# dcvan24/pivot-scheduling

Hardware: AMD Instinct MI355X
Metric: task x host placement candidates scored/sec (HBM GB/s % peak) at 1/2/4/8 MI355X (higher is better)
Workload: dtype f64; 1 GPU; synthetic 1000000 hosts x 10000 ready tasks per round, 20 zones, cost_aware best-fit, one independent scenario per GPU; scenarios_per_gpu=1, tasks_per_round=10000, zones=20, policy=ca_bf, parallelism=scenario-sharded x1 (no data-path collective)

## Files before the change

pivot-scheduling_amd/csrc/pvt_zwalk.hip:

```cpp
#include <hip/hip_runtime.h>
#include <stdint.h>

#include "pivot_place.h"
#include "pvt_device.h"
#include "pvt_kernels.h"
#include "pvt_zwin_dev.h"

namespace pvt {

constexpr int ZW_THREADS = 256;
constexpr int ZW_WAVES = ZW_THREADS / 64;
constexpr int ZW_SCAN = 8;
constexpr int ZW_MINB = ZW_MIN_PARTS;
constexpr int ZW_PR = 8;
constexpr double ZW_BIG = 0x1p500;

#ifndef PVT_ZW_UNROLL
#define PVT_ZW_UNROLL 8
#endif
#ifndef PVT_ZW_CF
#define PVT_ZW_CF 0
#endif
constexpr int ZW_UNROLL = PVT_ZW_UNROLL;
constexpr int ZW_SB = 64;
constexpr int32_t ZW_SAME = -1;
template <int WM>
struct ZwalkLDS {
  double wa[4][WM];
  int32_t wid[WM];
  int32_t wz[WM];
  uint64_t zm[WM / 64];
  double csum[ZMAX * ZMAX], bsum[ZMAX * ZMAX];
  int32_t cnt[ZW_SCAN][ZW_WAVES];
  double red[ZW_WAVES][12];
  double smin[ZW_SB][4];
  double lg[128][4];
  int32_t lgid[128];
  int32_t rwho[64], rstart[64];
  uint64_t sbits[CHAIN_MAX / 64];
  uint32_t amask[ZMAX];
  uint32_t umask;
  int32_t nwin, bail;
  int32_t touch[WM / 64];
};

__device__ __forceinline__ double nan_max(double a, double b) {
  return (a != a || b <= a) ? a : b;
}
__device__ __forceinline__ double wave_nmax_d(double v) {
  return wave_reduce_d(v, [](double a, double b) { return nan_max(a, b); });
}

__global__ __launch_bounds__(256) void host_min_kernel(const double* avail, int H, int lo, int hi,
                                                       double* part) {
  __shared__ double red[4][4];
  const int tid = threadIdx.x, lane = tid & 63, wave = tid >> 6;
  double m[4] = {DINF, DINF, DINF, DINF};
  for (int h = lo + blockIdx.x * 256 + tid; h < hi; h += gridDim.x * 256)
#pragma unroll
    for (int r = 0; r < 4; r++) m[r] = fmin(m[r], avail[(size_t)r * H + h]);
#pragma unroll
  for (int r = 0; r < 4; r++) {
    m[r] = wave_min_d(m[r]);
    if (lane == 0) red[wave][r] = m[r];
  }
  __syncthreads();
  if (tid < 4) {
    double v = red[0][tid];
    for (int w = 1; w < 4; w++) v = fmin(v, red[w][tid]);
    part[blockIdx.x * 4 + tid] = v;
  }
}

template <int N> struct IntC { static constexpr int value = N; };

constexpr int ZW_CAP = 128;
__device__ __forceinline__ int lowbit_exp(double v) {
  const uint64_t b = (uint64_t)__double_as_longlong(v);
  const uint64_t m = b & ((1ull << 52) - 1);
  const int e = (int)((b >> 52) & 0x7ff);
  if (e == 0) return m ? -1074 + __builtin_ctzll(m) : 4096;
  return (e - 1075) + __builtin_ctzll(m | (1ull << 52));
}
__device__ __forceinline__ int high_exp(double v) {
  return (int)(((uint64_t)__double_as_longlong(v) >> 52) & 0x7ff) - 1023;
}
template <bool STRICT>
__device__ __forceinline__ int copies_cf(double x, double d, bool& sure) {
  if (__double_as_longlong(d) == 0) return ZW_CAP;
  const double q = x * __builtin_amdgcn_rcp(d);
  double kf = STRICT ? __builtin_ceil(q) - 1.0 : __builtin_floor(q);
  kf = __builtin_fmin(kf, (double)ZW_CAP);
  const double e0 = __builtin_fma(-kf, d, x), e1 = __builtin_fma(-(kf + 1.0), d, x);
  const double big = __builtin_fabs(x) + (kf + 1.0) * d;
  const bool nice = high_exp(big) + 2 <= min(lowbit_exp(x), lowbit_exp(d)) + 53;
  const double err = nice ? 0.0 : (kf + 2.0) * 0x1p-52 * (big + d);
  const bool fit0 = STRICT ? (e0 > err) : (e0 >= err && (nice || e0 > err));
  const bool out1 = kf >= (double)ZW_CAP || (STRICT ? (e1 <= -err && (nice || e1 < -err)) : (e1 < -err));
  sure = sure && kf >= 1.0 && fit0 && out1 && (q == q);
  return (int)kf;
}

#define UNI(c) (__builtin_amdgcn_readfirstlane((int)(c)) != 0)

template <bool STRICT>
__device__ __forceinline__ bool fit_res(double m) { return STRICT ? (m > 0.0) : (m >= 0.0); }

__device__ __forceinline__ void wave_lds_sync() {
  __atomic_signal_fence(__ATOMIC_SEQ_CST);
  __builtin_amdgcn_s_waitcnt(0xc07f);
  __atomic_signal_fence(__ATOMIC_SEQ_CST);
}

template <int WM = ZW_M>
__device__ __forceinline__ void compact_zone_window(const int32_t* zone, int Z, uint32_t U,
                                                    int h_lo, int h_hi, int32_t* wid, int32_t* wz,
                                                    int32_t (*cnt)[ZW_WAVES], int32_t* nwin) {
  compact_zone_window_t<WM, ZW_THREADS, ZW_SCAN>(zone, Z, U, h_lo, h_hi, wid, wz, cnt, nwin);
}

#ifdef PVT_STAMPS
__device__ __forceinline__ uint64_t zstamp() {
  uint64_t t;
  __builtin_amdgcn_sched_barrier(0);
  asm volatile("s_memtime %0\n\ts_waitcnt lgkmcnt(0)" : "=s"(t)::"memory");
  __builtin_amdgcn_sched_barrier(0);
  return t;
}
#endif

template <bool KEYED, bool STRICT, bool FF = false, int WM = ZW_M, bool FAST = false>
__global__ __launch_bounds__(ZW_THREADS) void zwalk_kernel(ZwalkArgs A) {
  static_assert(!FF || (!KEYED && STRICT), "FF: chain mode, strict fit");
  static_assert(WM == ZW_M || !KEYED, "keyed / ordered / sharded windows: ZW_M hosts");
  __shared__ ZwalkLDS<WM> S;
#ifdef PVT_STAMPS
  const uint64_t t_start = zstamp();
  uint64_t n_chunks = 0, n_switch = 0, n_bulk = 0, n_runs = 0;
  uint64_t st_search = 0, st_p1 = 0, st_p2 = 0, n_probe = 0, n_iter = 0, st_batch = 0, n_single = 0;
  uint64_t st_setup = 0, st_loop = 0, st_who = 0, st_rep = 0;
  uint64_t n_cf = 0;
#endif
  const int b = blockIdx.x, tid = threadIdx.x, lane = tid & 63, wave = tid >> 6;
  const bool tabm = !KEYED && A.tab.nch > 0;
  const int base = KEYED ? 0 : tabm ? A.tab.coff[b] : A.coff[b];
  const int nt = KEYED ? A.knt : tabm ? A.tab.coff[b + 1] - A.tab.coff[b] : A.coff[b + 1] - base;
  const int32_t* gcmap = KEYED ? nullptr : A.cmap + base;
  auto cmap_at = [&](int i) -> int { return gcmap[i]; };
  const bool segm = !KEYED && (tabm || A.cseg);
  int32_t* status = A.status + 2 * b;
  const int Z = A.Z, H = A.H;
  auto report = [&](int s0, int s1) {
    status[0] = s0; status[1] = s1;
    if (!KEYED && A.hstat) { A.hstat[2 * b] = s0; A.hstat[2 * b + 1] = s1; }
  };

  auto publish_map = [&]() {
    if (tabm) {
      int32_t* wmap = const_cast<int32_t*>(A.cmap) + base;
      for (int k = A.tab.csoff[b]; k < A.tab.csoff[b + 1]; k++) {
        const int sg = A.tab.csegid[k], c0 = A.tab.seg_cstart[sg], o0 = A.tab.seg_off[sg];
        const int len = A.tab.seg_off[sg + 1] - o0;
        for (int i = tid; i < len; i += ZW_THREADS) wmap[c0 + i] = o0 + i;
      }
      if (b == 0) {
        const int ns = A.tab.nseg, nc = A.tab.nch;
        for (int i = tid; i <= ns; i += ZW_THREADS) {
          A.tab.o_seg_off[i] = A.tab.seg_off[i];
          if (i < ns) { A.tab.o_seg_chain[i] = A.tab.seg_chain[i]; A.tab.o_seg_cstart[i] = A.tab.seg_cstart[i]; }
        }
        for (int i = tid; i <= nc; i += ZW_THREADS) A.tab.o_coff[i] = A.tab.coff[i];
      }
    }
  };
  double mn[4];
  uint32_t U;
  int nwin;
#ifdef PVT_STAMPS
  uint64_t t_load, t_cert, t_win, t_cap;
#endif
  if constexpr (FAST) {
    static_assert(!KEYED && !FF && WM == ZW_M && ZW_M == 4 * ZW_THREADS, "fast prologue: best-fit chains");
    static_assert(ZW_ENT <= 64 && ZW_ENT <= ZW_SB, "entries: a lane each, in rwho / rstart / lg");
    const int j = min((int)A.cert.cwin[b], ZMAX - 1);
    const ZoneWindow* const zw = &A.zpre->w[j];
    const int ZZ = Z * Z;
    double cs[4], bs[4], ha[4];
#pragma unroll
    for (int u = 0; u < 4; u++) {
      const int i = tid + u * ZW_THREADS;
      cs[u] = i < ZZ ? A.csum[i] : 0.0;
      bs[u] = i < ZZ ? A.bsum[i] : 0.0;
    }
#pragma unroll
    for (int r = 0; r < 4; r++) ha[r] = A.hmin[tid * 4 + r];
    const uint32_t zu = A.zpre->U[j];
    const int zn = zw->n, zbad = zw->bad;
    int32_t wi[4], wzv[4];
    double wv[4][4];
#pragma unroll
    for (int u = 0; u < 4; u++) {
      const int p = tid + u * ZW_THREADS;
      wi[u] = zw->id[p];
      wzv[u] = zw->z[p];
#pragma unroll
      for (int r = 0; r < 4; r++) wv[u][r] = zw->a[r][p];
    }
    const int k0 = A.tab.csoff[b], k1 = A.tab.csoff[b + 1];
    double mxv = -DINF;
    bool badv = false;
    for (int k = k0 + wave; k < k1; k += ZW_WAVES) {
      const int sg = A.tab.csegid[k], c0 = A.tab.seg_cstart[sg];
      const int len = A.tab.seg_off[sg + 1] - A.tab.seg_off[sg];
      const GroupCert* const gc = A.cert.rec + min((int)A.cert.seg_grp[sg], GCOMPACT_MAX - 1);
      const int ne = (len + 63) >> 6, e = A.cert.seg_ent[sg] + lane;
      const bool on = lane < ne && lane < GC_SUB && e < ZW_ENT;
      double sm[4];
#pragma unroll
      for (int r = 0; r < 4; r++) sm[r] = on ? gc->smin[lane][r] : DINF;
      const double gm = lane < 4 ? gc->mx[lane] : -DINF;
      badv |= gc->bad != 0 || gc->n != len;
      mxv = fmax(mxv, gm);
      if (on) {
#pragma unroll
        for (int r = 0; r < 4; r++) S.lg[e][r] = sm[r];
        S.rstart[e] = c0 + 64 * lane;
        S.rwho[e] = c0 + min(64 * lane + 64, len);
      }
    }
    publish_map();
#pragma unroll
    for (int u = 0; u < 4; u++) {
      const int i = tid + u * ZW_THREADS;
      if (i < ZZ) { S.csum[i] = cs[u]; S.bsum[i] = bs[u]; }
    }
    if (tid < CHAIN_MAX / 64) S.sbits[tid] = 0;
    if (tid < WM / 64) S.touch[tid] = 0;
    if (tid < ZW_SB) {
#pragma unroll
      for (int r = 0; r < 4; r++) S.smin[tid][r] = -DINF;
    }
    nwin = min(zn, ZW_M);
#pragma unroll
    for (int u = 0; u < 4; u++) {
      const int p = tid + u * ZW_THREADS;
      if (p < nwin) {
        S.wid[p] = wi[u];
        S.wz[p] = wzv[u];
#pragma unroll
        for (int r = 0; r < 4; r++) S.wa[r][p] = wv[u][r];
      }
    }
#pragma unroll
    for (int r = 0; r < 4; r++) ha[r] = wave_min_d(ha[r]);
    const bool wbadv = __ballot(badv) != 0;
    if (lane < 4) S.red[wave][lane] = mxv;
    if (lane == 0) {
#pragma unroll
      for (int r = 0; r < 4; r++) S.red[wave][8 + r] = ha[r];
      S.cnt[0][wave] = wbadv ? 1 : 0;
    }
#ifdef PVT_STAMPS
    t_load = zstamp();
#endif
    __syncthreads();
    if (tid < Z) {
      uint32_t m = 0;
      for (int z = 0; z < Z; z++) m |= (S.csum[tid * Z + z] == 0.0) ? (1u << z) : 0u;
      S.amask[tid] = m;
    }
    for (int k = k0 + tid; k < k1; k += ZW_THREADS) {
      const int p = A.tab.seg_cstart[A.tab.csegid[k]];
      if (p > 0 && p < CHAIN_MAX) atomicOr(&S.sbits[p >> 6], 1ull << (p & 63));
    }
    double mx[4];
    bool bad = false;
#pragma unroll
    for (int w = 0; w < ZW_WAVES; w++) bad |= S.cnt[0][w] != 0;
#pragma unroll
    for (int r = 0; r < 4; r++) {
      mx[r] = fmax(fmax(S.red[0][r], S.red[1][r]), fmax(S.red[2][r], S.red[3][r]));
      ha[r] = fmin(fmin(S.red[0][8 + r], S.red[1][8 + r]), fmin(S.red[2][8 + r], S.red[3][8 + r]));
    }
    const int ne = min((int)A.cert.cent[b], ZW_ENT);
    {
      double v = lane < ne ? S.lg[lane][wave] : DINF;
#pragma unroll
      for (int off = 1; off < 64; off <<= 1) v = fmin(v, __shfl_down(v, off));
      if (lane < ne) {
        const int q = (S.rstart[lane] + 63) >> 6;
        if (q * 64 < S.rwho[lane] && q < ZW_SB) S.smin[q][wave] = v;
      }
      if (lane == 0) S.red[0][4 + wave] = v;
    }
    bool sep = false;
#pragma unroll
    for (int r = 0; r < 4; r++) sep |= (ha[r] - mx[r] >= 0x1p-288);
    U = zu;
    const bool cover = zu != 0 && (A.cert.cu[b] & ~zu) == 0;
    const bool stop = bad || !sep || nt <= 0 || nt > CHAIN_MAX || !cover || zbad != 0 || nwin <= 0;
#ifdef PVT_STAMPS
    t_cert = t_win = t_cap = zstamp();
#endif
    __syncthreads();
    if (tid == 0) {
      int cert = stop ? 0 : ZW_CERT_FAST;
#pragma unroll
      for (int r = 0; r < 4; r++) {
        const double mnr = S.red[0][4 + r];
        cert |= ((mx[r] <= 0.0 && mnr >= 0.0) ? (1 << r) : 0) | ((ha[r] >= 0x1p-287) ? (16 << r) : 0);
      }
      if (A.hcert) A.hcert[b] = cert;
      if (stop) report(0, nt <= 0 ? 0 : 1);
    }
    if (A.cmax && tid < 4) A.cmax[b * 4 + tid] = mx[tid];
    if (stop) return;
  } else {
    static_assert(ZMAX * ZMAX <= 4 * ZW_THREADS && ZW_MINB == ZW_THREADS, "prologue loads");
    const int ZZ = KEYED ? 0 : Z * Z;
    double cs[4], bs[4];
#pragma unroll
    for (int u = 0; u < 4; u++) {
      const int i = tid + u * ZW_THREADS;
      cs[u] = i < ZZ ? A.csum[i] : 0.0;
      bs[u] = i < ZZ ? A.bsum[i] : 0.0;
    }
    double ha[4] = {FF ? -DINF : DINF, FF ? -DINF : DINF, FF ? -DINF : DINF, FF ? -DINF : DINF};
    if (!KEYED) {
#pragma unroll
      for (int r = 0; r < 4; r++) {
        const double x = A.hmin[tid * 4 + r];
        ha[r] = FF ? nan_max(ha[r], x) : fmin(ha[r], x);
      }
    }
    publish_map();
    int wv[ZW_PR];
    if (tabm) {
      const int k0 = A.tab.csoff[b], k1 = A.tab.csoff[b + 1];
#pragma unroll
      for (int u = 0; u < ZW_PR; u++) {
        const int i = u * ZW_THREADS + tid;
        int v = -1;
        for (int k = k0; k < k1; k++) {
          const int sg = A.tab.csegid[k], c0 = A.tab.seg_cstart[sg];
          if (i >= c0) v = A.tab.seg_off[sg] + (i - c0);
        }
        wv[u] = i < nt ? v : -1;
      }
    } else {
#pragma unroll
      for (int u = 0; u < ZW_PR; u++) {
        const int i = u * ZW_THREADS + tid;
        wv[u] = i < nt ? (KEYED ? i : gcmap[i]) : -1;
      }
    }
    const int sg0 = tabm ? A.tab.csoff[b] : (!KEYED && A.cseg) ? A.csoff[b] : 0;
    const int sg1 = tabm ? A.tab.csoff[b + 1] : (!KEYED && A.cseg) ? A.csoff[b + 1] : 0;
    const uint32_t zpu = (!KEYED && WM == ZW_M && A.zpre && lane < Z) ? A.zpre->U[lane] : 0u;

#pragma unroll
    for (int u = 0; u < 4; u++) {
      const int i = tid + u * ZW_THREADS;
      if (i < ZZ) { S.csum[i] = cs[u]; S.bsum[i] = bs[u]; }
    }
    if (tid == 0) { S.umask = 0; S.nwin = 0; S.bail = 0; }
    if (tid < CHAIN_MAX / 64) S.sbits[tid] = 0;
    if (tid < WM / 64) S.touch[tid] = 0;
#ifdef PVT_STAMPS
    t_load = zstamp();
#endif
    __syncthreads();
    if (!KEYED && tid < Z) {
      uint32_t m = 0;
      for (int z = 0; z < Z; z++) m |= (S.csum[tid * Z + z] == 0.0) ? (1u << z) : 0u;
      S.amask[tid] = m;
    }
    if (tabm) {
      for (int k = sg0 + tid; k < sg1; k += ZW_THREADS) {
        const int p = A.tab.seg_cstart[A.tab.csegid[k]];
        if (p > 0 && p < CHAIN_MAX) atomicOr(&S.sbits[p >> 6], 1ull << (p & 63));
      }
    } else {
      for (int k = sg0 + tid; k < sg1; k += ZW_THREADS) {
        const int p = A.cseg[k];
        if (p > 0 && p < CHAIN_MAX) atomicOr(&S.sbits[p >> 6], 1ull << (p & 63));
      }
    }

    uint32_t abits = 0;
    double mx[4] = {-DINF, -DINF, -DINF, -DINF};
    mn[0] = mn[1] = mn[2] = mn[3] = DINF;
    bool bad = false;
    for (int i0 = 0; i0 < nt; i0 += ZW_PR * ZW_THREADS) {
      int av[ZW_PR], wn[ZW_PR];
      double dv[ZW_PR][4];
#pragma unroll
      for (int u = 0; u < ZW_PR; u++) {
        const int w = max(wv[u], 0);
        av[u] = A.anc[w];
#pragma unroll
        for (int r = 0; r < 4; r++) dv[u][r] = A.dem[(size_t)w * 4 + r];
      }
#pragma unroll
      for (int u = 0; u < ZW_PR; u++) {
        const int i = i0 + ZW_PR * ZW_THREADS + u * ZW_THREADS + tid;
        wn[u] = i < nt ? (KEYED ? i : cmap_at(i)) : -1;
      }
#pragma unroll
      for (int u = 0; u < ZW_PR; u++) {
        const bool ok = wv[u] >= 0;
        double bm[4];
#pragma unroll
        for (int r = 0; r < 4; r++) bm[r] = ok ? dv[u][r] : DINF;
        if (ok) {
          const int a = av[u];
          if (a < 0 || a >= Z) {
            bad = true;
          } else {
            abits |= 1u << a;
#pragma unroll
            for (int r = 0; r < 4; r++) {
              bad |= !(__builtin_fabs(dv[u][r]) <= ZW_BIG);
              mx[r] = fmax(mx[r], dv[u][r]);
              mn[r] = fmin(mn[r], dv[u][r]);
            }
          }
        }
        const int blk = (i0 + u * ZW_THREADS) / 64 + wave;
        if (blk < ZW_SB - 1 && blk * 64 < nt) {
#pragma unroll
          for (int r = 0; r < 4; r++) bm[r] = wave_min_d(bm[r]);
          if (lane == 0) {
#pragma unroll
            for (int r = 0; r < 4; r++) S.smin[blk][r] = bm[r];
          }
        }
      }
#pragma unroll
      for (int u = 0; u < ZW_PR; u++) wv[u] = wn[u];
    }
    __syncthreads();
    uint32_t um = 0;
    if (!KEYED)
      for (uint32_t m = abits; m; m &= m - 1) um |= S.amask[__builtin_ctz(m)];
#pragma unroll
    for (int r = 0; r < 4; r++) {
      mx[r] = wave_max_d(mx[r]);
      mn[r] = wave_min_d(mn[r]);
      ha[r] = FF ? wave_nmax_d(ha[r]) : wave_min_d(ha[r]);
    }
    if (lane == 0) {
#pragma unroll
      for (int r = 0; r < 4; r++) { S.red[wave][r] = mx[r]; S.red[wave][4 + r] = mn[r]; S.red[wave][8 + r] = ha[r]; }
    }
    if (bad) S.bail = 1;
    if (um) atomicOr(&S.umask, um);
    __syncthreads();
#ifdef PVT_STAMPS
    t_cert = zstamp();
#endif
#pragma unroll
    for (int r = 0; r < 4; r++) {
      for (int w = 1; w < ZW_WAVES; w++) {
        mx[r] = fmax(mx[r], S.red[w][r]);
        mn[r] = fmin(mn[r], S.red[w][4 + r]);
        ha[r] = FF ? nan_max(ha[r], S.red[w][8 + r]) : fmin(ha[r], S.red[w][8 + r]);
      }
      mx[r] = fmax(mx[r], S.red[0][r]);
      mn[r] = fmin(mn[r], S.red[0][4 + r]);
      ha[r] = FF ? nan_max(ha[r], S.red[0][8 + r]) : fmin(ha[r], S.red[0][8 + r]);
    }
    if (!KEYED && A.cmax && tid < 4) A.cmax[b * 4 + tid] = mx[tid];
    if (!KEYED && A.hcert && tid == 0) {
      int cert = 0;
      if (!FF) {
#pragma unroll
        for (int r = 0; r < 4; r++)
          cert |= ((mx[r] <= 0.0 && mn[r] >= 0.0) ? (1 << r) : 0) | ((ha[r] >= 0x1p-287) ? (16 << r) : 0);
      }
      A.hcert[b] = cert;
    }
    bool sep = KEYED;
    if (FF) {
      sep = true;
#pragma unroll
      for (int r = 0; r < 4; r++) sep &= (ha[r] <= 0x1p298) && (mn[r] >= 0.0);
    } else {
#pragma unroll
      for (int r = 0; r < 4; r++) sep |= (ha[r] - mx[r] >= 0x1p-288);
    }
    U = S.umask;
    if (S.bail || !sep || nt <= 0 || (!KEYED && nt > CHAIN_MAX)) {
      if (tid == 0) report(0, (KEYED || nt <= 0) ? 0 : 1);
      return;
    }
    const FrontierSlot* pw = A.pwin ? A.pwin + (KEYED ? 0 : b) : nullptr;
    const ZoneWindow* zw = nullptr;
    if (!KEYED && WM == ZW_M && !pw && A.zpre && U != 0) {
      const uint64_t cover = __ballot(zpu != 0 && (U & ~zpu) == 0);
      if (cover) {
        const int j = __builtin_ctzll(cover);
        zw = &A.zpre->w[j];
        U = (uint32_t)__builtin_amdgcn_readlane((int)zpu, j);
      }
    }
    if (pw) {
      const int nw = min(pw->n, ZW_M);
      for (int p = tid; p < nw; p += ZW_THREADS) {
        const int32_t h = pw->id[p];
        S.wid[p] = h;
        S.wz[p] = KEYED ? 0 : A.zone[h];
      }
      if (tid == 0) S.nwin = nw;
      __syncthreads();
    } else if (zw) {
      const int nw = min(zw->n, ZW_M);
      for (int p = tid; p < nw; p += ZW_THREADS) { S.wid[p] = zw->id[p]; S.wz[p] = zw->z[p]; }
      if (tid == 0) S.nwin = nw;
      __syncthreads();
    } else if (KEYED) {
      const int nw = min(A.kn_dev ? *A.kn_dev : A.kn, ZW_M);
      for (int p = tid; p < nw; p += ZW_THREADS) { S.wid[p] = A.lo + A.kperm[p]; S.wz[p] = 0; }
      if (tid == 0) S.nwin = nw;
      __syncthreads();
    } else {
      compact_zone_window<WM>(A.zone, Z, U, 0, H, S.wid, S.wz, S.cnt, &S.nwin);
    }
    nwin = S.nwin;
#ifdef PVT_STAMPS
    t_win = zstamp();
#endif
    bool wbad = false;
    ZwUndo* const ud = (!KEYED && A.undo) ? A.undo + b : nullptr;
    if (ud && tid == 0) ud->count = nwin;
    static_assert(WM <= ZW_MBIG, "ZwUndo holds every window");
    static_assert(WM % (4 * ZW_THREADS) == 0, "window capacities: four hosts per thread per pass");
    for (int p0 = 0; p0 < WM && p0 < nwin; p0 += 4 * ZW_THREADS) {
      double v[4][4];
#pragma unroll
      for (int u = 0; u < 4; u++) {
        const int p = p0 + u * ZW_THREADS + tid;
        const int h = p < nwin ? S.wid[p] : 0;
#pragma unroll
        for (int r = 0; r < 4; r++)
          v[u][r] = p >= nwin ? 0.0 : (pw ? pw->a[r][p] : zw ? zw->a[r][p] : A.avail[(size_t)r * H + h]);
      }
#pragma unroll
      for (int u = 0; u < 4; u++) {
        const int p = p0 + u * ZW_THREADS + tid;
        if (p < nwin) {
#pragma unroll
          for (int r = 0; r < 4; r++) {
            wbad |= !(__builtin_fabs(v[u][r]) <= ZW_BIG);
            S.wa[r][p] = v[u][r];
          }
          if (ud) {
            ud->id[p] = S.wid[p];
#pragma unroll
            for (int r = 0; r < 4; r++) ud->a[r][p] = v[u][r];
          }
        }
      }
    }
    if (wbad) S.bail = 1;
    __syncthreads();
#ifdef PVT_STAMPS
    t_cap = zstamp();
#endif
    if (S.bail || nwin == 0) {
      if (tid == 0) report(0, KEYED ? 0 : 1);
      return;
    }
    const int nsb = min((nt + 63) >> 6, ZW_SB);
    for (int blk = ZW_SB - 1 + wave; blk < nsb; blk += ZW_WAVES) {
      const int i1 = blk == ZW_SB - 1 ? nt : min(nt, blk * 64 + 64);
      double bm[4] = {DINF, DINF, DINF, DINF};
      for (int i = blk * 64 + lane; i < i1; i += 64) {
        const int w = KEYED ? i : cmap_at(i);
#pragma unroll
        for (int r = 0; r < 4; r++) bm[r] = fmin(bm[r], A.dem[(size_t)w * 4 + r]);
      }
#pragma unroll
      for (int r = 0; r < 4; r++) bm[r] = wave_min_d(bm[r]);
      if (lane == 0) {
#pragma unroll
        for (int r = 0; r < 4; r++) S.smin[blk][r] = bm[r];
      }
    }
    __syncthreads();
    static_assert(ZW_SB == 64 && ZW_WAVES == 4, "suffix minima: one wave per dimension, a lane per batch");
    {
      double v = lane < nsb ? S.smin[lane][wave] : DINF;
#pragma unroll
      for (int off = 1; off < 64; off <<= 1) v = fmin(v, __shfl_down(v, off));
      if (lane < nsb) S.smin[lane][wave] = v;
    }
    __syncthreads();
  }
  if (wave != 0) return;
#ifdef PVT_STAMPS
  const uint64_t t_walk = zstamp();
#endif

  const int nch = (nwin + 63) >> 6;
  int p0 = 0;
  int cur = -1;
  int done = 0;
  bool failed = false, exhausted = false;
  double ra0, ra1, ra2, ra3;
  int32_t rid;
  uint64_t rzm = 0, rvalid = 0;
  bool dirty = false;
  auto load_chunk = [&](int c) {
    const int p = c * 64 + lane;
    const int q = min(p, nwin - 1);
    ra0 = S.wa[0][q]; ra1 = S.wa[1][q]; ra2 = S.wa[2][q]; ra3 = S.wa[3][q];
    rid = S.wid[q];
    rvalid = __ballot(p < nwin);
    dirty = false;
    __builtin_amdgcn_s_waitcnt(0xc07f);
  };
  auto store_chunk = [&](int c) {
    const int p = c * 64 + lane;
    if (dirty && p < nwin) { S.wa[0][p] = ra0; S.wa[1][p] = ra1; S.wa[2][p] = ra2; S.wa[3][p] = ra3; }
    dirty = false;
  };
  double rb0 = 0.0, rb1 = 0.0, rb2 = 0.0, rb3 = 0.0;
  int32_t bid = 0;
  uint64_t bzm = 0, bvalid = 0;
  bool bdirty = false;
  int pb = -1;
  auto load_b = [&](int c) {
    bdirty = false;
    if (c >= nch) { pb = -1; bvalid = 0; bzm = 0; return; }
    pb = c;
    const int p = c * 64 + lane;
    const int q = min(p, nwin - 1);
    rb0 = S.wa[0][q]; rb1 = S.wa[1][q]; rb2 = S.wa[2][q]; rb3 = S.wa[3][q];
    bid = S.wid[q];
    bvalid = __ballot(p < nwin);
    bzm = cur >= 0 ? rfl_u64(S.zm[c]) : 0;
    __builtin_amdgcn_s_waitcnt(0xc07f);
  };
  auto store_b = [&]() {
    const int p = pb * 64 + lane;
    if (bdirty && pb >= 0 && p < nwin) { S.wa[0][p] = rb0; S.wa[1][p] = rb1; S.wa[2][p] = rb2; S.wa[3][p] = rb3; }
    bdirty = false;
  };
  auto run_bulk = [&](auto cft, double& c0, double& c1, double& c2, double& c3, int32_t cid, double d0,
                      double d1, double d2, double d3, uint64_t m0, int R, int k) -> int {
#ifdef PVT_STAMPS
    const uint64_t tA = zstamp();
#endif
    if (!(d0 >= 0.0 && d1 >= 0.0 && d2 >= 0.0 && d3 >= 0.0)) R = 1;
    const bool on1 = __builtin_amdgcn_inverse_ballot_w64(m0);
    const bool two = __double_as_longlong(d2) == 0 && __double_as_longlong(d3) == 0;
    R = __builtin_amdgcn_readfirstlane(R);
    int cnt = 0;
#ifdef PVT_STAMPS
    const uint64_t tA1 = zstamp();
    st_setup += tA1 - tA;
#endif
    bool cf = false;
#if PVT_ZW_CF
    if (decltype(cft)::value && R >= 2) {
      bool sure = true;
      int k = ZW_CAP;
      if (on1) {
        k = min(copies_cf<STRICT>(c0, d0, sure), copies_cf<STRICT>(c1, d1, sure));
        if (!two) k = min(k, min(copies_cf<STRICT>(c2, d2, sure), copies_cf<STRICT>(c3, d3, sure)));
      }
      const bool bad = on1 && !sure;
      const uint64_t ub = __ballot(bad);
      const int kc = on1 && sure ? k : 0;
      const int inc = wave_incl_scan_dpp(kc);
      const int first_bad = ub ? __builtin_ctzll(ub) : 64;
      const int before_bad = first_bad == 0 ? 0 : __builtin_amdgcn_readlane(inc, first_bad - 1);
      cf = ub == 0 || before_bad >= R;
      if (cf) cnt = (lane < first_bad) ? kc : 0;
#ifdef PVT_STAMPS
      n_cf += cf;
#endif
    }
#endif
    if (!cf) {
      double x0 = on1 ? c0 : -DINF, x1 = on1 ? c1 : -DINF, x2 = on1 ? c2 : -DINF, x3 = on1 ? c3 : -DINF;
      int t = 0;
      auto pass1 = [&](auto dims) {
        constexpr int D = decltype(dims)::value;
        int u = __builtin_ctzll(m0), fb = 0;
        for (;;) {
          t = __builtin_amdgcn_readfirstlane(t);
          u = __builtin_amdgcn_readfirstlane(u);
          fb = __builtin_amdgcn_readfirstlane(fb);
          bool f = false;
#pragma unroll
          for (int j = 1; j <= ZW_UNROLL; j++) {
            x0 -= d0; x1 -= d1;
            if (D == 4) { x2 -= d2; x3 -= d3; }
            f = fit_res<STRICT>(D == 4 ? fmin(fmin(x0, x1), fmin(x2, x3)) : fmin(x0, x1));
            cnt = f ? t + j : cnt;
          }
          t += ZW_UNROLL;
          const uint64_t an = __ballot(f);
          if (UNI(an == 0)) break;
          const int un = __builtin_ctzll(an);
          if (un != u) {
            u = un;
            fb = __builtin_amdgcn_readlane(wave_incl_scan_dpp(cnt), u - 1);
          }
          if (UNI(fb + t >= R)) break;
        }
      };
      if (two) pass1(IntC<2>{});
      else pass1(IntC<4>{});
#ifdef PVT_STAMPS
      n_iter += t;
#endif
    }
#ifdef PVT_STAMPS
    st_loop += zstamp() - tA1;
#endif
    const int incl = wave_incl_scan_dpp(cnt);
    const int pre = incl - cnt;
    const int asg = max(0, min(cnt, R - pre));
    const int covered = min(R, __builtin_amdgcn_readlane(incl, 63));
#ifdef PVT_STAMPS
    const uint64_t tB = zstamp();
    st_p1 += tB - tA;
#endif
    if (asg > 0) S.lgid[k + pre] = cid;
    const int amax = wave_max_i32(asg);
#ifdef PVT_STAMPS
    const uint64_t tC = zstamp();
    st_who += tC - tB;
#endif
    if (two) {
      for (int m = 0; m < amax; m += 4) {
#pragma unroll
        for (int u = 0; u < 4; u++) {
          const double o = m + u < asg ? -1.0 : -0.0;
          c0 = __builtin_fma(o, d0, c0);
          c1 = __builtin_fma(o, d1, c1);
        }
      }
    } else {
      for (int m = 0; m < amax; m += 4) {
#pragma unroll
        for (int u = 0; u < 4; u++) {
          const double o = m + u < asg ? -1.0 : -0.0;
          c0 = __builtin_fma(o, d0, c0);
          c1 = __builtin_fma(o, d1, c1);
          c2 = __builtin_fma(o, d2, c2);
          c3 = __builtin_fma(o, d3, c3);
        }
      }
    }
#ifdef PVT_STAMPS
    st_rep += zstamp() - tC;
#endif
    if (asg > 0) {
      const int q = k + pre + asg - 1;
      S.lg[q][0] = c0; S.lg[q][1] = c1; S.lg[q][2] = c2; S.lg[q][3] = c3;
    }
#ifdef PVT_STAMPS
    st_p2 += zstamp() - tB;
#endif
    return covered;
  };
  load_chunk(0);
  load_b(1);
  auto task_at = [&](int i) { return i < nt ? (KEYED ? i : cmap_at(i)) : 0; };
  int nw = task_at(lane);
  double nd0 = A.dem[(size_t)nw * 4 + 0], nd1 = A.dem[(size_t)nw * 4 + 1];
  double nd2 = A.dem[(size_t)nw * 4 + 2], nd3 = A.dem[(size_t)nw * 4 + 3];
  int nanc = A.anc[nw], ncal = A.ord[nw];
  int nw1 = task_at(64 + lane);
  int carry = 0;
  int fk = 0, ftw = 0, fcal = 0;
  int32_t fprev = 0;
  S.lgid[lane] = ZW_SAME;
  S.lgid[64 + lane] = ZW_SAME;
  auto flush_log = [&]() {
    if (UNI(fk > 0)) {
      const int32_t raw = S.lgid[lane];
      const uint64_t upto = __ballot(raw != ZW_SAME) & (lane == 63 ? ~0ull : ((2ull << lane) - 1ull));
      const int32_t from = __shfl(raw, upto ? 63 - __builtin_clzll(upto) : 0);
      const int32_t id = upto ? from : fprev;
      fprev = __builtin_amdgcn_readlane(id, 63);
      if (lane < fk) {
        WinRec& e = A.wlog[ftw];
        e.s = 0.0;
        e.id = id;
        e.a[0] = S.lg[lane][0]; e.a[1] = S.lg[lane][1]; e.a[2] = S.lg[lane][2]; e.a[3] = S.lg[lane][3];
        A.placement[fcal] = id;
      }
    }
  };
  for (int i0 = 0; UNI(i0 < nt && !failed); i0 += 64) {
#ifdef PVT_STAMPS
    uint64_t tb0 = zstamp();
#endif
#pragma unroll
    for (int r = 0; r < 4; r++) mn[r] = S.smin[min(i0 >> 6, ZW_SB - 1)][r];
    const int tw = nw;
    const double td[4] = {nd0, nd1, nd2, nd3};
    const int tanc = nanc;
    const int tcal = ncal;
    __atomic_signal_fence(__ATOMIC_SEQ_CST);
    __builtin_amdgcn_s_waitcnt(0x0f70);
    __atomic_signal_fence(__ATOMIC_SEQ_CST);
    flush_log();
    if (i0 + 64 < nt) {
      nw = nw1;
      nd0 = A.dem[(size_t)nw * 4 + 0]; nd1 = A.dem[(size_t)nw * 4 + 1];
      nd2 = A.dem[(size_t)nw * 4 + 2]; nd3 = A.dem[(size_t)nw * 4 + 3];
      nanc = A.anc[nw]; ncal = A.ord[nw];
      nw1 = task_at(i0 + 128 + lane);
    }
    const int kn = min(64, nt - i0);
    bool uni = __ballot(lane < kn && tanc != cur) == 0;
    uint64_t E;
    {
      bool same = lane > 0 && lane < kn;
#pragma unroll
      for (int r = 0; r < 4; r++)
        same &= __double_as_longlong(__shfl_up(td[r], 1)) == __double_as_longlong(td[r]);
      E = __ballot(same);
      if (segm) E &= ~rfl_u64(S.sbits[i0 >> 6]);
    }
    int extc = -1;
    auto ext_len = [&]() -> int {
      if (extc < 0) {
        extc = 0;
        if (kn == 64 && i0 + 64 < nt && uni) {
          const int kn2 = min(64, nt - i0 - 64);
          const double l0 = readlane_d(td[0], 63), l1 = readlane_d(td[1], 63);
          const double l2 = readlane_d(td[2], 63), l3 = readlane_d(td[3], 63);
          bool eq = lane < kn2 && readlane_i(tanc, 63) == nanc &&
                    __double_as_longlong(nd0) == __double_as_longlong(l0) &&
                    __double_as_longlong(nd1) == __double_as_longlong(l1) &&
                    __double_as_longlong(nd2) == __double_as_longlong(l2) &&
                    __double_as_longlong(nd3) == __double_as_longlong(l3);
          if (segm) eq = eq && !((rfl_u64(S.sbits[(i0 >> 6) + 1]) >> lane) & 1ull);
          const uint64_t m = __ballot(eq);
          extc = m == ~0ull ? 64 : __builtin_ctzll(~m);
        }
        extc = __builtin_amdgcn_readfirstlane(extc);
      }
      return extc;
    };
    auto run_len = [&](int k) {
      int r = k < 63 ? min(kn - k, 1 + __builtin_ctzll(~(E >> (k + 1)))) : 1;
      if (k + r == 64) r = min(64, r + ext_len());
      return r;
    };
    auto run_step = [&](int k) -> int {
#ifdef PVT_STAMPS
      const uint64_t t0 = zstamp();
#define ZW_SEARCH_DONE() (st_search += zstamp() - t0)
#else
#define ZW_SEARCH_DONE() ((void)0)
#endif
      const double d0 = readlane_d(td[0], k), d1 = readlane_d(td[1], k);
      const double d2 = readlane_d(td[2], k), d3 = readlane_d(td[3], k);
      const int R = run_len(k);
      for (;;) {
        const double n0 = ra0 - d0, n1 = ra1 - d1, n2 = ra2 - d2, n3 = ra3 - d3;
        uint64_t fm = __ballot(fit_res<STRICT>(fmin(fmin(n0, n1), fmin(n2, n3)))) & rvalid;
        if (FF) fm &= rzm;
        if (!FF && UNI((fm & ~rzm) != 0)) return 0;
        if (UNI(fm != 0)) {
          dirty = true;
          ZW_SEARCH_DONE();
          return run_bulk(IntC<0>{}, ra0, ra1, ra2, ra3, rid, d0, d1, d2, d3, fm, R, k);
        }
        if (__ballot(((rvalid >> lane) & 1ull) && fits<STRICT>(ra0, ra1, ra2, ra3, mn[0], mn[1], mn[2], mn[3])))
          break;
        if (p0 + 1 >= nch) return 0;
        store_b();
        store_chunk(p0);
        ++p0;
        rzm = rfl_u64(S.zm[p0]);
        load_chunk(p0);
        load_b(p0 + 1);
      }
      if (pb >= 0) {
        const double q0 = rb0 - d0, q1 = rb1 - d1, q2 = rb2 - d2, q3 = rb3 - d3;
        uint64_t fb = __ballot(fit_res<STRICT>(fmin(fmin(q0, q1), fmin(q2, q3)))) & bvalid;
        if (FF) fb &= bzm;
        if (!FF && UNI((fb & ~bzm) != 0)) return 0;
        if (UNI(fb != 0)) {
          bdirty = true;
          ZW_SEARCH_DONE();
          return run_bulk(IntC<0>{}, rb0, rb1, rb2, rb3, bid, d0, d1, d2, d3, fb, R, k);
        }
      }
      for (int c = (pb >= 0 ? pb : p0) + 1; c < nch; c++) {
        const int p = c * 64 + lane;
        const int q = min(p, nwin - 1);
        double x0 = S.wa[0][q], x1 = S.wa[1][q], x2 = S.wa[2][q], x3 = S.wa[3][q];
        const int32_t xid = S.wid[q];
        const uint64_t xzm = rfl_u64(S.zm[c]);
#ifdef PVT_STAMPS
        n_probe++;
#endif
        uint64_t fm = __ballot(p < nwin && fit_res<STRICT>(fmin(fmin(x0 - d0, x1 - d1),
                                                                fmin(x2 - d2, x3 - d3))));
        if (FF) fm &= xzm;
        if (!FF && UNI((fm & ~xzm) != 0)) return 0;
        if (UNI(fm != 0)) {
          ZW_SEARCH_DONE();
          const int got = run_bulk(IntC<0>{}, x0, x1, x2, x3, xid, d0, d1, d2, d3, fm, R, k);
          if (p < nwin) { S.wa[0][p] = x0; S.wa[1][p] = x1; S.wa[2][p] = x2; S.wa[3][p] = x3; }
          if (!KEYED && lane == 0) S.touch[c] = 1;
          return got;
        }
      }
      ZW_SEARCH_DONE();
      return 0;
    };
#undef ZW_SEARCH_DONE
#ifdef PVT_STAMPS
    st_batch += zstamp() - tb0;
#endif
    int k = carry;
    {
      wave_lds_sync();
      const int32_t cid = lane < carry ? S.lgid[64 + lane] : ZW_SAME;
      if (lane < carry) {
#pragma unroll
        for (int r = 0; r < 4; r++) S.lg[lane][r] = S.lg[64 + lane][r];
      }
      S.lgid[lane] = cid;
      S.lgid[64 + lane] = ZW_SAME;
      wave_lds_sync();
    }
    while (UNI(k < kn)) {
      k = __builtin_amdgcn_readfirstlane(k);
      p0 = __builtin_amdgcn_readfirstlane(p0);
      pb = __builtin_amdgcn_readfirstlane(pb);
      done = __builtin_amdgcn_readfirstlane(done);
      rzm = rfl_u64(rzm);
      bzm = rfl_u64(bzm);
      if (uni) {
        for (; k < kn;) {
          k = __builtin_amdgcn_readfirstlane(k);
          const double d0 = readlane_d(td[0], k), d1 = readlane_d(td[1], k);
          const double d2 = readlane_d(td[2], k), d3 = readlane_d(td[3], k);
          const double n0 = ra0 - d0, n1 = ra1 - d1, n2 = ra2 - d2, n3 = ra3 - d3;
          const uint64_t fm0 = __ballot(fit_res<STRICT>(fmin(fmin(n0, n1), fmin(n2, n3)))) & rvalid;
          const uint64_t m0 = fm0 & rzm;
          if (UNI(m0 == 0 || (!FF && (fm0 & ~rzm) != 0))) break;
          const int R = run_len(k);
          if (UNI(R >= 2)) {
            const int c = run_bulk(IntC<1>{}, ra0, ra1, ra2, ra3, rid, d0, d1, d2, d3, m0, R, k);
            k += c;
            done += c;
            dirty = true;
#ifdef PVT_STAMPS
            n_chunks += c;
            n_bulk += c;
            n_runs++;
#endif
            continue;
          }
          const bool win = __builtin_amdgcn_inverse_ballot_w64(m0 & (0ull - m0));
          ra0 = win ? n0 : ra0; ra1 = win ? n1 : ra1; ra2 = win ? n2 : ra2; ra3 = win ? n3 : ra3;
          if (win) {
            S.lg[k][0] = n0; S.lg[k][1] = n1; S.lg[k][2] = n2; S.lg[k][3] = n3;
            S.lgid[k] = rid;
          }
          dirty = true;
#ifdef PVT_STAMPS
          n_chunks++;
          n_single++;
#endif
          done++;
          k++;
        }
        if (UNI(k >= kn)) break;
        const int got = run_step(k);
        if (UNI(got > 0)) {
          k += got;
          done += got;
#ifdef PVT_STAMPS
          n_chunks += got;
          n_bulk += got;
          n_runs++;
#endif
          continue;
        }
      }
      const double d0 = readlane_d(td[0], k), d1 = readlane_d(td[1], k);
      const double d2 = readlane_d(td[2], k), d3 = readlane_d(td[3], k);
      const int a = uni ? cur : readlane_i(tanc, k);
      if (a != cur) {
        bool ok = true;
        if (!KEYED && lane < Z) {
          const double c = S.csum[a * Z + lane], bw = S.bsum[a * Z + lane];
          if (c == 0.0) ok = bw > 0.0;
          else if (FF || !((U >> lane) & 1u)) ok = (c >= 0x1p-300) && (bw > 0.0) && (bw <= 0x1p300);
        }
        if (__ballot(!ok)) { failed = true; break; }
        const uint32_t am = KEYED ? ~0u : S.amask[a];
        for (int c = 0; c < nch; c++) {
          const int p = c * 64 + lane;
          const uint64_t m = __ballot(p < nwin && (KEYED || ((am >> S.wz[min(p, nwin - 1)]) & 1u)));
          if (lane == 0) S.zm[c] = m;
          if (c == p0) rzm = m;
          if (c == pb) bzm = m;
        }
        cur = a;
        uni = __ballot(lane >= k && lane < kn && tanc != cur) == 0;
        __builtin_amdgcn_s_waitcnt(0xc07f);
#ifdef PVT_STAMPS
        n_switch++;
#endif
      }
      auto zero_exact = [&](bool f, bool k0, double a0, double a1, double a2, double a3, int q) {
        if (FF) return k0;
        if (__builtin_expect(__ballot(f && !k0) != 0, 0)) {
          if (f && !k0) {
            const int z = S.wz[q];
            const double s2 = norm2_seq(a0 - d0, a1 - d1, a2 - d2, a3 - d3);
            const double sc = (S.csum[a * Z + z] * __builtin_sqrt(s2)) / S.bsum[a * Z + z];
            k0 = __double_as_longlong(sc) == 0;
          }
        }
        return k0;
      };
      const double n0 = ra0 - d0, n1 = ra1 - d1, n2 = ra2 - d2, n3 = ra3 - d3;
      const uint64_t fm0 = __ballot(fit_res<STRICT>(fmin(fmin(n0, n1), fmin(n2, n3)))) & rvalid;
      bool found = true;
#ifdef PVT_STAMPS
      n_chunks++;
#endif
      const uint64_t m0 = fm0 & rzm;
      if (__builtin_expect(m0 != 0 && (FF || (fm0 & ~rzm) == 0), 1)) {
        const bool win = __builtin_amdgcn_inverse_ballot_w64(m0 & (0ull - m0));
        ra0 = win ? n0 : ra0; ra1 = win ? n1 : ra1; ra2 = win ? n2 : ra2; ra3 = win ? n3 : ra3;
        if (win) {
          S.lg[k][0] = n0; S.lg[k][1] = n1; S.lg[k][2] = n2; S.lg[k][3] = n3;
          S.lgid[k] = rid;
        }
        dirty = true;
      } else {
        bool inb = false;
        if (fm0 == 0 && pb >= 0) {
          const double q0 = rb0 - d0, q1 = rb1 - d1, q2 = rb2 - d2, q3 = rb3 - d3;
          const uint64_t fb = __ballot(fit_res<STRICT>(fmin(fmin(q0, q1), fmin(q2, q3)))) & bvalid;
          const uint64_t mb = fb & bzm;
          if (mb != 0 && (FF || (fb & ~bzm) == 0)) {
            const bool win = __builtin_amdgcn_inverse_ballot_w64(mb & (0ull - mb));
            rb0 = win ? q0 : rb0; rb1 = win ? q1 : rb1; rb2 = win ? q2 : rb2; rb3 = win ? q3 : rb3;
            if (win) {
              S.lg[k][0] = q0; S.lg[k][1] = q1; S.lg[k][2] = q2; S.lg[k][3] = q3;
              S.lgid[k] = bid;
            }
            bdirty = true;
            inb = true;
          }
        }
        if (!inb) {
          found = false;
          store_b();
          double g0 = n0, g1 = n1, g2 = n2, g3 = n3;
          uint64_t fm = fm0, m = fm0 & rzm;
#ifdef PVT_STAMPS
          for (int pass = 0;; pass++) {
            n_chunks += pass > 0;
#else
          for (;;) {
#endif
            if (fm & ~rzm)
              m = __ballot(zero_exact((fm >> lane) & 1ull, (rzm >> lane) & 1ull, ra0, ra1, ra2,
                                      ra3, min(p0 * 64 + lane, nwin - 1))) & fm;
            if (m) {
              const bool win = lane == __builtin_ctzll(m);
              ra0 = win ? g0 : ra0; ra1 = win ? g1 : ra1; ra2 = win ? g2 : ra2; ra3 = win ? g3 : ra3;
              if (win) {
                S.lg[k][0] = g0; S.lg[k][1] = g1; S.lg[k][2] = g2; S.lg[k][3] = g3;
                S.lgid[k] = rid;
              }
              dirty = true;
              found = true;
              break;
            }
            if (__ballot(((rvalid >> lane) & 1ull) && fits<STRICT>(ra0, ra1, ra2, ra3, mn[0], mn[1], mn[2], mn[3])))
              break;
            store_chunk(p0);
            if (++p0 >= nch) break;
            rzm = rfl_u64(S.zm[p0]);
            load_chunk(p0);
            g0 = ra0 - d0; g1 = ra1 - d1; g2 = ra2 - d2; g3 = ra3 - d3;
            fm = __ballot(fit_res<STRICT>(fmin(fmin(g0, g1), fmin(g2, g3)))) & rvalid;
            m = fm & rzm;
          }
          if (!found && p0 < nch) {
            store_chunk(p0);
            for (int c = p0 + 1; c < nch; c++) {
#ifdef PVT_STAMPS
              n_chunks++;
#endif
              const int p = c * 64 + lane;
              const int q = min(p, nwin - 1);
              const double a0 = S.wa[0][q], a1 = S.wa[1][q], a2 = S.wa[2][q], a3 = S.wa[3][q];
              const int32_t id = S.wid[q];
              const uint64_t zm = rfl_u64(S.zm[c]);
              const bool f = p < nwin && fits<STRICT>(a0, a1, a2, a3, d0, d1, d2, d3);
              const bool k0 = zero_exact(f, (zm >> lane) & 1ull, a0, a1, a2, a3, q);
              const uint64_t mc = __ballot(f && k0);
              if (mc) {
                if (lane == __builtin_ctzll(mc)) {
                  const double c0 = a0 - d0, c1 = a1 - d1, c2 = a2 - d2, c3 = a3 - d3;
                  S.wa[0][q] = c0; S.wa[1][q] = c1; S.wa[2][q] = c2; S.wa[3][q] = c3;
                  S.lg[k][0] = c0; S.lg[k][1] = c1; S.lg[k][2] = c2; S.lg[k][3] = c3;
                  S.lgid[k] = id;
                  if (!KEYED) S.touch[c] = 1;
                }
                found = true;
                break;
              }
            }
          }
          wave_lds_sync();
          load_b(p0 + 1);
        }
      }
      if (UNI(!found)) {
        failed = true;
        exhausted = nwin >= WM;
        break;
      }
      done++;
      k++;
    }
#ifdef PVT_STAMPS
    tb0 = zstamp();
#endif
    fk = __builtin_amdgcn_readfirstlane(k);
    ftw = tw;
    fcal = tcal;
    carry = __builtin_amdgcn_readfirstlane(k > kn ? k - kn : 0);
#ifdef PVT_STAMPS
    st_batch += zstamp() - tb0;
#endif
  }
  flush_log();
  if (KEYED) {
    store_chunk(p0);
    store_b();
    wave_lds_sync();
    for (int p = lane; p < nwin; p += 64) {
      const int h = S.wid[p];
#pragma unroll
      for (int r = 0; r < 4; r++) A.wb[(size_t)r * H + h] = S.wa[r][p];
    }
  }
  if (!KEYED && A.undo && !failed && done == nt) {
    store_chunk(p0);
    store_b();
    wave_lds_sync();
    const int top = max(p0, pb);
    for (int c = 0; c < nch; c++) {
      if (c > top && !S.touch[c]) continue;
      const int p = c * 64 + lane;
      if (p < nwin) {
        const int h = S.wid[p];
#pragma unroll
        for (int r = 0; r < 4; r++) A.wb[(size_t)r * H + h] = S.wa[r][p];
      }
    }
  }
  if (lane == 0) report(done, (failed && !KEYED) ? (exhausted ? 2 : 1) : 0);
#ifdef PVT_STAMPS
  if (lane == 0 && A.stamps) {
    const uint64_t t_end = zstamp();
    atomicAdd((unsigned long long*)&A.stamps[0], (unsigned long long)(t_walk - t_start));
    atomicAdd((unsigned long long*)&A.stamps[1], (unsigned long long)(t_end - t_walk));
    atomicAdd((unsigned long long*)&A.stamps[2], (unsigned long long)n_chunks);
    atomicAdd((unsigned long long*)&A.stamps[3], (unsigned long long)done);
    atomicAdd((unsigned long long*)&A.stamps[4], (unsigned long long)n_switch);
    atomicAdd((unsigned long long*)&A.stamps[5], (unsigned long long)n_bulk);
    atomicAdd((unsigned long long*)&A.stamps[6], (unsigned long long)n_runs);
    atomicAdd((unsigned long long*)&A.stamps[7], (unsigned long long)st_search);
    atomicAdd((unsigned long long*)&A.stamps[8], (unsigned long long)st_p1);
    atomicAdd((unsigned long long*)&A.stamps[9], (unsigned long long)st_p2);
    atomicAdd((unsigned long long*)&A.stamps[10], (unsigned long long)n_probe);
    atomicAdd((unsigned long long*)&A.stamps[11], (unsigned long long)n_iter);
    atomicAdd((unsigned long long*)&A.stamps[12], (unsigned long long)st_batch);
    atomicAdd((unsigned long long*)&A.stamps[13], (unsigned long long)n_single);
    atomicAdd((unsigned long long*)&A.stamps[20], (unsigned long long)(t_cert - t_start));
    atomicAdd((unsigned long long*)&A.stamps[21], (unsigned long long)(t_win - t_cert));
    atomicAdd((unsigned long long*)&A.stamps[22], (unsigned long long)(t_cap - t_win));
    atomicAdd((unsigned long long*)&A.stamps[23], (unsigned long long)(t_walk - t_cap));
    atomicAdd((unsigned long long*)&A.stamps[24], (unsigned long long)st_setup);
    atomicAdd((unsigned long long*)&A.stamps[25], (unsigned long long)st_loop);
    atomicAdd((unsigned long long*)&A.stamps[26], (unsigned long long)st_who);
    atomicAdd((unsigned long long*)&A.stamps[27], (unsigned long long)st_rep);
    atomicAdd((unsigned long long*)&A.stamps[28], (unsigned long long)n_cf);
    atomicAdd((unsigned long long*)&A.stamps[29], (unsigned long long)(t_load - t_start));
  }
#endif
}

void launch_host_min(const double* avail, int H, int lo, int hi, double* part, hipStream_t st) {
  PVT_LAUNCH(host_min_kernel, dim3(ZW_MINB), dim3(256), 0, st, avail, H, lo, hi, part);
}

void launch_zwalk(const ZwalkArgs& a, int nchains, hipStream_t st) {
  if (a.cert.fast && a.tab.nch > 0 && a.zpre && !a.pwin)
    PVT_LAUNCH((zwalk_kernel<false, false, false, ZW_M, true>), dim3(nchains), dim3(ZW_THREADS), 0, st, a);
  else
    PVT_LAUNCH((zwalk_kernel<false, false>), dim3(nchains), dim3(ZW_THREADS), 0, st, a);
}
void launch_zwalk_big(const ZwalkArgs& a, int nchains, hipStream_t st) {
  PVT_LAUNCH((zwalk_kernel<false, false, false, ZW_MBIG>), dim3(nchains), dim3(ZW_THREADS), 0, st, a);
}
void launch_zwalk_ff(const ZwalkArgs& a, int nchains, hipStream_t st) {
  PVT_LAUNCH((zwalk_kernel<false, true, true>), dim3(nchains), dim3(ZW_THREADS), 0, st, a);
}

__global__ __launch_bounds__(256) void host_absmax_kernel(const double* avail, int H, int lo, int hi,
                                                          double* part) {
  __shared__ double red[4][4];
  const int tid = threadIdx.x, lane = tid & 63, wave = tid >> 6;
  double m[4] = {0.0, 0.0, 0.0, 0.0};
  for (int h = lo + blockIdx.x * 256 + tid; h < hi; h += gridDim.x * 256)
#pragma unroll
    for (int r = 0; r < 4; r++) {
      m[r] = nan_max(m[r], __builtin_fabs(avail[(size_t)r * H + h]));
    }
#pragma unroll
  for (int r = 0; r < 4; r++) {
    m[r] = wave_nmax_d(m[r]);
    if (lane == 0) red[wave][r] = m[r];
  }
  __syncthreads();
  if (tid < 4) {
    double v = red[0][tid];
    for (int w = 1; w < 4; w++) v = nan_max(v, red[w][tid]);
    part[blockIdx.x * 4 + tid] = v;
  }
}
void launch_host_absmax(const double* avail, int H, int lo, int hi, double* part, hipStream_t st) {
  PVT_LAUNCH(host_absmax_kernel, dim3(ZW_MINB), dim3(256), 0, st, avail, H, lo, hi, part);
}
void launch_zwalk_keyed(const ZwalkArgs& a, bool strict, hipStream_t st) {
  if (strict) PVT_LAUNCH((zwalk_kernel<true, true>), dim3(1), dim3(ZW_THREADS), 0, st, a);
  else PVT_LAUNCH((zwalk_kernel<true, false>), dim3(1), dim3(ZW_THREADS), 0, st, a);
}

__global__ __launch_bounds__(1024) void dem_min_kernel(const double* dem, int n, double* out) {
  __shared__ double red[16][4];
  const int tid = threadIdx.x, lane = tid & 63, wave = tid >> 6;
  double m[4] = {DINF, DINF, DINF, DINF};
  for (int i = tid; i < n; i += 1024)
#pragma unroll
    for (int r = 0; r < 4; r++) m[r] = fmin(m[r], dem[(size_t)i * 4 + r]);
#pragma unroll
  for (int r = 0; r < 4; r++) {
    m[r] = wave_min_d(m[r]);
    if (lane == 0) red[wave][r] = m[r];
  }
  __syncthreads();
  if (tid < 4) {
    double v = red[0][tid];
    for (int w = 1; w < 16; w++) v = fmin(v, red[w][tid]);
    out[tid] = v;
  }
}
__global__ void alive_flags_kernel(const double* avail, int H, int lo, int hs, const double* dmin,
                                   int strict, uint8_t* flags) {
  const int h = lo + blockIdx.x * blockDim.x + threadIdx.x;
  if (h >= hs) return;
  const double a0 = avail[h], a1 = avail[(size_t)H + h], a2 = avail[2 * (size_t)H + h],
               a3 = avail[3 * (size_t)H + h];
  flags[h - lo] = strict ? fits<true>(a0, a1, a2, a3, dmin[0], dmin[1], dmin[2], dmin[3])
                    : fits<false>(a0, a1, a2, a3, dmin[0], dmin[1], dmin[2], dmin[3]);
}
void launch_alive_flags(const double* avail, int H, int lo, int hs, const double* dem, int n,
                        int strict, double* dmin, uint8_t* flags, hipStream_t st) {
  PVT_LAUNCH(dem_min_kernel, dim3(1), dim3(1024), 0, st, dem, n, dmin);
  if (hs <= lo) return;
  PVT_LAUNCH(alive_flags_kernel, dim3((hs - lo + 255) / 256), dim3(256), 0, st, avail, H,
                     lo, hs, dmin, strict, flags);
}


__global__ __launch_bounds__(ZW_THREADS) void zwin_build_kernel(ZwinArgs A) {
  __shared__ uint32_t amask[ZMAX];
  __shared__ uint32_t umask;
  __shared__ int32_t cnt[ZW_SCAN][ZW_WAVES];
  __shared__ int32_t nwin;
  const int b = blockIdx.x, tid = threadIdx.x, Z = A.Z;
  FrontierSlot* out = A.out + b;
  if (tid == 0) { umask = 0; nwin = 0; }
  if (tid < Z) {
    uint32_t m = 0;
    for (int z = 0; z < Z; z++) m |= (A.csum[tid * Z + z] == 0.0) ? (1u << z) : 0u;
    amask[tid] = m;
  }
  __syncthreads();
  uint32_t um = 0;
  for (int i = A.coff[b] + tid; i < A.coff[b + 1]; i += ZW_THREADS) {
    const int a = A.anc[A.cmap[i]];
    if (a >= 0 && a < Z) um |= amask[a];
  }
  if (um) atomicOr(&umask, um);
  __syncthreads();
  compact_zone_window(A.zone, Z, umask, A.lo, A.hi, out->id, nullptr, cnt, &nwin);
  const int n = nwin;
  for (int p = tid; p < n; p += ZW_THREADS) {
    const int h = out->id[p];
#pragma unroll
    for (int r = 0; r < 4; r++) out->a[r][p] = A.avail[(size_t)r * A.H + h];
  }
  if (tid == 0) { out->n = n; out->total = n; }
}

__global__ __launch_bounds__(256) void zwin_gather_kernel(const double* avail, int H, int lo,
                                                          const int32_t* perm, const int32_t* count,
                                                          FrontierSlot* out) {
  const int c = *count, n = min(c, ZW_M);
  for (int p = threadIdx.x; p < n; p += 256) {
    const int h = lo + perm[p];
    out->id[p] = h;
#pragma unroll
    for (int r = 0; r < 4; r++) out->a[r][p] = avail[(size_t)r * H + h];
  }
  if (threadIdx.x == 0) { out->n = n; out->total = c; }
}

__global__ __launch_bounds__(256) void zwin_merge_kernel(const uint8_t* pkgs, int64_t pkg_bytes,
                                                         int world, int nslots, FrontierSlot* out,
                                                         double* hmin) {
  __shared__ int32_t off[PVT_SHARD_MAX_WORLD + 1];
  const int b = blockIdx.x, tid = threadIdx.x;
  auto hdr = [&](int k) { return reinterpret_cast<const FrontierHdr*>(pkgs + (size_t)k * pkg_bytes); };
  if (b == nslots) {
    for (int i = tid; hmin && i < ZW_MIN_PARTS * 4; i += 256) {
      double m = DINF;
      for (int k = 0; k < world; k++) m = fmin(m, (&hdr(k)->hmin[0][0])[i]);
      (&hmin[0])[i] = m;
    }
    return;
  }
  auto slot = [&](int k) { return reinterpret_cast<const FrontierSlot*>(hdr(k) + 1) + b; };
  if (tid == 0) {
    int o = 0, tot = 0;
    for (int k = 0; k < world; k++) { off[k] = o; o += slot(k)->n; tot += slot(k)->total; }
    off[world] = o;
    out[b].n = min(o, ZW_M);
    out[b].total = tot;
  }
  __syncthreads();
  for (int k = 0; k < world && off[k] < ZW_M; k++) {
    const FrontierSlot* s = slot(k);
    const int n = min(s->n, ZW_M - off[k]);
    for (int p = tid; p < n; p += 256) {
      const int q = off[k] + p;
      out[b].id[q] = s->id[p];
#pragma unroll
      for (int r = 0; r < 4; r++) out[b].a[r][q] = s->a[r][p];
    }
  }
}

void launch_zwin_build(const ZwinArgs& a, int nchains, hipStream_t st) {
  PVT_LAUNCH(zwin_build_kernel, dim3(nchains), dim3(ZW_THREADS), 0, st, a);
}
void launch_zwin_gather(const double* avail, int H, int lo, const int32_t* perm,
                        const int32_t* count, FrontierSlot* out, hipStream_t st) {
  PVT_LAUNCH(zwin_gather_kernel, dim3(1), dim3(256), 0, st, avail, H, lo, perm, count, out);
}
void launch_zwin_merge(const uint8_t* pkgs, int64_t pkg_bytes, int world, int nslots,
                       FrontierSlot* out, double* hmin, hipStream_t st) {
  PVT_LAUNCH(zwin_merge_kernel, dim3(nslots + 1), dim3(256), 0, st, pkgs, pkg_bytes, world,
                     nslots, out, hmin);
}

}
```

Baseline: 57300 billion candidates/s.

## Snapshot remaining capacity during fit scan to skip most of the replay loop

```diff
diff --git a/pivot-scheduling_amd/csrc/pvt_zwalk.hip b/pivot-scheduling_amd/csrc/pvt_zwalk.hip
--- a/pivot-scheduling_amd/csrc/pvt_zwalk.hip
+++ b/pivot-scheduling_amd/csrc/pvt_zwalk.hip
@@ -140,6 +140,7 @@
   uint64_t st_search = 0, st_p1 = 0, st_p2 = 0, n_probe = 0, n_iter = 0, st_batch = 0, n_single = 0;
   uint64_t st_setup = 0, st_loop = 0, st_who = 0, st_rep = 0;
   uint64_t n_cf = 0;
+  uint64_t n_part = 0, s_pasg = 0, n_fromc = 0, n_rep = 0;
 #endif
   const int b = blockIdx.x, tid = threadIdx.x, lane = tid & 63, wave = tid >> 6;
   const bool tabm = !KEYED && A.tab.nch > 0;
@@ -662,6 +663,8 @@
     st_setup += tA1 - tA;
 #endif
     bool cf = false;
+    double s0 = c0, s1 = c1, s2 = c2, s3 = c3;
+    int t = 0;
 #if PVT_ZW_CF
     if (decltype(cft)::value && R >= 2) {
       bool sure = true;
@@ -685,31 +688,49 @@
 #endif
     if (!cf) {
       double x0 = on1 ? c0 : -DINF, x1 = on1 ? c1 : -DINF, x2 = on1 ? c2 : -DINF, x3 = on1 ? c3 : -DINF;
-      int t = 0;
       auto pass1 = [&](auto dims) {
         constexpr int D = decltype(dims)::value;
+        constexpr int U = ZW_UNROLL;
         int u = __builtin_ctzll(m0), fb = 0;
+        bool f = false;
         for (;;) {
           t = __builtin_amdgcn_readfirstlane(t);
           u = __builtin_amdgcn_readfirstlane(u);
           fb = __builtin_amdgcn_readfirstlane(fb);
-          bool f = false;
-#pragma unroll
-          for (int j = 1; j <= ZW_UNROLL; j++) {
-            x0 -= d0; x1 -= d1;
-            if (D == 4) { x2 -= d2; x3 -= d3; }
-            f = fit_res<STRICT>(D == 4 ? fmin(fmin(x0, x1), fmin(x2, x3)) : fmin(x0, x1));
-            cnt = f ? t + j : cnt;
+          if (t > 0) {
+            s0 = f ? x0 : s0; s1 = f ? x1 : s1;
+            if (D == 4) { s2 = f ? x2 : s2; s3 = f ? x3 : s3; }
           }
+          double a0[U], a1[U], a2[U], a3[U], mp[U], mq[U], mm[U];
+#pragma unroll
+          for (int j = 0; j < U + 3; j++) {
+            if (j < U) {
+              a0[j] = (j ? a0[j - 1] : x0) - d0;
+              a1[j] = (j ? a1[j - 1] : x1) - d1;
+              if (D == 4) { a2[j] = (j ? a2[j - 1] : x2) - d2; a3[j] = (j ? a3[j - 1] : x3) - d3; }
+            }
+            if (j >= 1 && j - 1 < U) {
+              mp[j - 1] = fmin(a0[j - 1], a1[j - 1]);
+              if (D == 4) mq[j - 1] = fmin(a2[j - 1], a3[j - 1]);
+            }
+            if (j >= 2 && j - 2 < U) mm[j - 2] = D == 4 ? fmin(mp[j - 2], mq[j - 2]) : mp[j - 2];
+            if (j >= 3) {
+              f = fit_res<STRICT>(mm[j - 3]);
+              cnt += f ? 1 : 0;
+            }
+            __builtin_amdgcn_sched_barrier(0);
+          }
+          x0 = a0[U - 1]; x1 = a1[U - 1];
+          if (D == 4) { x2 = a2[U - 1]; x3 = a3[U - 1]; }
           t += ZW_UNROLL;
-          const uint64_t an = __ballot(f);
-          if (UNI(an == 0)) break;
+          const uint64_t an = rfl_u64(__ballot(f));
+          if (an == 0) break;
           const int un = __builtin_ctzll(an);
           if (un != u) {
             u = un;
             fb = __builtin_amdgcn_readlane(wave_incl_scan_dpp(cnt), u - 1);
           }
-          if (UNI(fb + t >= R)) break;
+          if (fb + t >= R) break;
         }
       };
       if (two) pass1(IntC<2>{});
@@ -730,30 +751,61 @@
     st_p1 += tB - tA;
 #endif
     if (asg > 0) S.lgid[k + pre] = cid;
-    const int amax = wave_max_i32(asg);
-#ifdef PVT_STAMPS
+    const int sbc = min(cnt / ZW_UNROLL * ZW_UNROLL, max(t - ZW_UNROLL, 0));
+#ifdef PVT_ZW_REPLAY_FULL
+    const bool snap = false;
+#else
+    const bool snap = asg >= sbc;
+#endif
+    const int nrep = snap ? asg - sbc : asg;
+    c0 = snap ? s0 : c0; c1 = snap ? s1 : c1;
+    c2 = snap ? s2 : c2; c3 = snap ? s3 : c3;
+    const uint64_t over = rfl_u64(__ballot(asg > 0 && !snap));
+#ifdef PVT_ZW_REPLAY_FULL
+    (void)over;
+    const int nmax = wave_max_i32(asg);
+#else
+    int nmax = rfl_u64(__ballot(snap && nrep > 4)) ? ZW_UNROLL : rfl_u64(__ballot(snap && nrep > 0)) ? 4 : 0;
+    if (over) nmax = max(nmax, __builtin_amdgcn_readlane(asg, __builtin_ctzll(over)));
+#if PVT_ZW_CF
+    if (cf) nmax = wave_max_i32(asg);
+#endif
+#endif
+#ifdef PVT_STAMPS
+    {
+      const uint64_t part = __ballot(asg > 0 && asg < cnt);
+      n_part += part != 0;
+      if (part) s_pasg += (uint64_t)__builtin_amdgcn_readlane(asg, __builtin_ctzll(part));
+      n_fromc += over != 0;
+    }
     const uint64_t tC = zstamp();
     st_who += tC - tB;
 #endif
     if (two) {
-      for (int m = 0; m < amax; m += 4) {
+      for (int m = 0; m < nmax; m += 4) {
 #pragma unroll
         for (int u = 0; u < 4; u++) {
-          const double o = m + u < asg ? -1.0 : -0.0;
+          const double o = m + u < nrep ? -1.0 : -0.0;
           c0 = __builtin_fma(o, d0, c0);
           c1 = __builtin_fma(o, d1, c1);
         }
+#ifdef PVT_STAMPS
+        n_rep += 4;
+#endif
       }
     } else {
-      for (int m = 0; m < amax; m += 4) {
+      for (int m = 0; m < nmax; m += 4) {
 #pragma unroll
         for (int u = 0; u < 4; u++) {
-          const double o = m + u < asg ? -1.0 : -0.0;
+          const double o = m + u < nrep ? -1.0 : -0.0;
           c0 = __builtin_fma(o, d0, c0);
           c1 = __builtin_fma(o, d1, c1);
           c2 = __builtin_fma(o, d2, c2);
           c3 = __builtin_fma(o, d3, c3);
         }
+#ifdef PVT_STAMPS
+        n_rep += 4;
+#endif
       }
     }
 #ifdef PVT_STAMPS
@@ -1191,6 +1243,10 @@
     atomicAdd((unsigned long long*)&A.stamps[11], (unsigned long long)n_iter);
     atomicAdd((unsigned long long*)&A.stamps[12], (unsigned long long)st_batch);
     atomicAdd((unsigned long long*)&A.stamps[13], (unsigned long long)n_single);
+    atomicAdd((unsigned long long*)&A.stamps[14], (unsigned long long)n_part);
+    atomicAdd((unsigned long long*)&A.stamps[15], (unsigned long long)s_pasg);
+    atomicAdd((unsigned long long*)&A.stamps[30], (unsigned long long)n_fromc);
+    atomicAdd((unsigned long long*)&A.stamps[31], (unsigned long long)n_rep);
     atomicAdd((unsigned long long*)&A.stamps[20], (unsigned long long)(t_cert - t_start));
     atomicAdd((unsigned long long*)&A.stamps[21], (unsigned long long)(t_win - t_cert));
     atomicAdd((unsigned long long*)&A.stamps[22], (unsigned long long)(t_cap - t_win));
```

After: 60100 billion candidates/s, median of 6. +4.9%, better.
